# NVIDIA-NeMo/NeMo

Hardware: AMD Instinct MI355X
Metric: audio-sec/s training throughput, Conformer-CTC-Large @ 1/2/4/8 MI355X (higher is better)
Workload: dtype bf16; 1 GPU; Conformer-CTC-Large bf16, batch=32x20s synthetic 16 kHz clips per GPU, 1xMI355X (BASELINE.json configs[1]); global_batch=32, parallelism=dp1

## Files before the change

### nemo_amd/csrc/attention.hip

```cpp
#include <stdlib.h>
#include "common.h"
#include "mi355x_asr.h"

typedef __attribute__((address_space(3))) void lds_void_t;
typedef const __attribute__((address_space(1))) void glb_void_t;
typedef __attribute__((ext_vector_type(4))) short s16x4;
typedef __attribute__((address_space(3))) s16x4 lds_s16x4_t;

typedef __attribute__((address_space(3))) const char lds_cchar_t;
__device__ __forceinline__ uint32_t lds_addr(const void* p) { return (uint32_t)(uintptr_t)(lds_cchar_t*)p; }

__device__ __forceinline__ void dma16(const void* src, const void* lds_base) {
  asm volatile("s_mov_b32 m0, %1\n\ts_nop 0\n\tglobal_load_lds_dwordx4 %0, off"
               :
               : "v"(src), "s"(__builtin_amdgcn_readfirstlane(lds_addr(lds_base)))
               : "memory");
}

__device__ __forceinline__ void dma4(const void* src, const void* lds_base) {
  asm volatile("s_mov_b32 m0, %1\n\ts_nop 0\n\tglobal_load_lds_dword %0, off"
               :
               : "v"(src), "s"(__builtin_amdgcn_readfirstlane(lds_addr(lds_base)))
               : "memory");
}

#define ABQ 128
#define ABK 32
#define ABAND (ABQ + ABK)
#define SG_LD 66
#define APRING 6

__device__ __forceinline__ uint32_t attn_key(const DropCfg& d, int b, int h) {
  return mix32(mix32(d.key ^ (uint32_t)(b * 0x632BE5AB)) + (uint32_t)h * 0x9E3779B9u);
}
#define ADROP_G 0x9E3779B9u
#define ADROP_KA 0x2C1B3Du
#define ADROP_KB 0x5A2D39u
__device__ __forceinline__ uint32_t adrop_rcode(uint32_t akey, uint32_t bi) { return mix32(akey + bi * 0x9E3779B9u); }
__device__ __forceinline__ uint32_t adrop_ccode(uint32_t bj) { return mix32(bj * 0x85EBCA6Bu + 0x165667B1u); }
__device__ __forceinline__ uint32_t adrop_seed(uint32_t x) { return __umul24(x, 0x846CA7u) + (x >> 13); }
__device__ __forceinline__ uint32_t adrop_y(uint32_t t) { return t ^ (t >> 15); }
__device__ __forceinline__ bool attn_keep(const DropCfg& d, uint32_t akey, int i, int j) {
  if (d.threshold == 0u) return true;
  const uint32_t seed = adrop_seed(adrop_rcode(akey, (uint32_t)i >> 2) ^ adrop_ccode((uint32_t)j >> 2));
  const uint32_t y = adrop_y(seed + (uint32_t)((i & 3) * 2 + ((j & 3) >> 1)) * ADROP_G);
  return __umul24(y, (j & 1) ? ADROP_KB : ADROP_KA) >= d.threshold;
}
__device__ __forceinline__ float attn_drop(const DropCfg& d, uint32_t akey, int i, int j) {
  return attn_keep(d, akey, i, j) ? d.scale : 0.f;
}

template <int ADK>
__device__ __forceinline__ int a_off(int r, int chunk) { return r * ADK + ((chunk ^ ((r >> 1) & 7)) << 3); }

template <int ADK>
__device__ __forceinline__ void stage_rows(const bf16_t* base, long long ld, int row0, int rmax, bf16_t* lds, int nchunks) {
  constexpr int NCH = ADK / 8;
  const int wave = threadIdx.x >> 6;
  for (int q0 = 0; q0 < nchunks; q0 += 256) {
    const int q = q0 + threadIdx.x;
    if (q0 + wave * 64 < nchunks) {
      const int r = q / NCH, ck = q % NCH;
      const int gck = ck ^ ((r >> 1) & 7);
      int gr = row0 + r;
      gr = gr < 0 ? 0 : (gr > rmax ? rmax : gr);
      const bf16_t* src = base + __mul24(gr, (int)ld) + gck * 8;
      bf16_t* dst = lds + (q0 + wave * 64) * 8;
      dma16(src, dst);
    }
  }
}
template <int ADK>
__device__ __forceinline__ void stage_v(const bf16_t* base, long long ld, int row0, int rmax, bf16_t* lds) {
  constexpr int NCH = ADK / 8;
  const int wave = threadIdx.x >> 6;
#pragma unroll
  for (int q0 = 0; q0 < 32 * NCH; q0 += 256) {
    const int q = q0 + threadIdx.x;
    const int k = q / NCH, cp = q % NCH;
    const int c = cp ^ ((k & 3) << 1);
    int gr = row0 + k;
    gr = gr > rmax ? rmax : gr;
    const bf16_t* src = base + __mul24(gr, (int)ld) + c * 8;
    bf16_t* dst = lds + (q0 + wave * 64) * 8;
    dma16(src, dst);
  }
}
template <int ADK>
__device__ __forceinline__ bf16x8 vt_frag(const bf16_t* vt, int dv0, int s, int lane) {
  const int t = lane & 15, g4 = (lane >> 4) & 1, lh = lane >> 5;
  const int col = dv0 + g4 * 16 + (t & 3) * 4;
  union { bf16x8 v; s16x4 h[2]; } u;
#pragma unroll
  for (int r = 0; r < 2; ++r) {
    const int krow = 16 * s + 8 * r + 4 * lh + (t >> 2);
    const int off = krow * ADK + (((col >> 3) ^ ((krow & 3) << 1)) << 3) + (col & 7);
    u.h[r] = __builtin_amdgcn_ds_read_tr16_b64_v4i16((lds_s16x4_t*)(vt + off));
  }
  return u.v;
}

__device__ __forceinline__ bf16x8 pack8(const float* v) {
  union { bf16x8 v; uint32_t w[4]; } u;
#pragma unroll
  for (int j = 0; j < 4; ++j) u.w[j] = pack_bf2(v[2 * j], v[2 * j + 1]);
  return u.v;
}

template <int NKK>
__device__ __forceinline__ void load_q(const bf16_t* qrow, const float* bias, bf16x8 (&out)[NKK], bool valid, int lh) {
#pragma unroll
  for (int kk = 0; kk < NKK; ++kk) {
    float v[8];
    const int k0 = kk * 16 + lh * 8;
    if (valid) {
      const u32x4 t = *reinterpret_cast<const u32x4*>(qrow + k0);
#pragma unroll
      for (int j = 0; j < 4; ++j) { v[2 * j] = __uint_as_float(t[j] << 16); v[2 * j + 1] = __uint_as_float(t[j] & 0xffff0000u); }
#pragma unroll
      for (int j = 0; j < 8; ++j) v[j] += bias[k0 + j];
    } else {
#pragma unroll
      for (int j = 0; j < 8; ++j) v[j] = 0.f;
    }
    out[kk] = pack8(v);
  }
}

template <int ADK>
__global__ __launch_bounds__(256, ADK == 64 ? 2 : 1) void relpos_flash_fwd_kernel(const bf16_t* __restrict__ qkv, long long ldq,
                                                                  const bf16_t* __restrict__ pos, long long ldp,
                                                                  const float* __restrict__ bias_u, const float* __restrict__ bias_v,
                                                                  const long long* __restrict__ len, bf16_t* __restrict__ ctx,
                                                                  bf16_t* __restrict__ ctx_lo, long long ldo,
                                                                  float* __restrict__ lse, int B, int H, int T,
                                                                  int Tp, float scale, DropCfg drop,
                                                                  const long long* __restrict__ cu) {
  drop_resolve(drop);
  constexpr int NKK = ADK / 16, NDT = ADK / 32, NCH = ADK / 8;
  __shared__ __attribute__((aligned(16))) bf16_t s_k2[2][ABK * ADK];
  __shared__ __attribute__((aligned(16))) bf16_t s_v2[2][ABK * ADK];
  __shared__ __attribute__((aligned(16))) bf16_t s_p[APRING * 32 * ADK];
  __shared__ __attribute__((aligned(16))) float s_g[4][32 * SG_LD];

  const int b = blockIdx.z, h = blockIdx.y;
  const int i0_blk = blockIdx.x * ABQ;
  const int lane = threadIdx.x & 63, wave = __builtin_amdgcn_readfirstlane(threadIdx.x >> 6);
  const int q = lane & 31, lh = lane >> 5;
  const int i = i0_blk + wave * 32 + q;
  const int L = (int)min((long long)T, len[b]);
  const bool qvalid = i < L;
  const int P = 2 * T - 1;
  const long long row0 = cu ? cu[b] : (long long)b * T;
  const int Tr = cu ? L : T;
  const int Trc = Tr > 0 ? Tr - 1 : 0;

  if (cu && i0_blk >= L) {
    if (lse && lh == 0 && i < T) lse[((long long)b * H + h) * T + i] = 0.f;
    return;
  }
  const bf16_t* qbase = qkv + row0 * ldq + h * ADK;
  const bf16_t* kbase = qbase + (ldq / 3);
  const bf16_t* vbase = qbase + 2 * (ldq / 3);
  const bf16_t* pbase = pos + h * ADK;

  bf16x8 qu[NKK], qv[NKK];
  load_q<NKK>(qbase + (long long)(i < Tr ? i : Trc) * ldq, bias_u + h * ADK, qu, i < Tr, lh);
  load_q<NKK>(qbase + (long long)(i < Tr ? i : Trc) * ldq, bias_v + h * ADK, qv, i < Tr, lh);

  f32x16 o[NDT];
#pragma unroll
  for (int t = 0; t < NDT; ++t)
#pragma unroll
    for (int r = 0; r < 16; ++r) o[t][r] = 0.f;
  float m_run = -INFINITY, l_run = 0.f;
  float* sg = s_g[wave];
  const uint32_t akey = attn_key(drop, b, h);
  const uint32_t arow = adrop_rcode(akey, (uint32_t)i >> 2), erow = (uint32_t)(i & 3) * (2u * ADROP_G);
  const float c2 = scale * 1.4426950408889634f, tau = 8.f / c2;

  const int nkt = (L + ABK - 1) / ABK;
  const int c0 = T - 1 - (i0_blk + ABQ - 1);
  if (nkt > 0) {
    stage_rows<ADK>(kbase, ldq, 0, Trc, s_k2[0], ABK * NCH);
    stage_v<ADK>(vbase, ldq, 0, Trc, s_v2[0]);
    stage_rows<ADK>(pbase, ldp, c0, P - 1, s_p, ABAND * NCH);
  }
  for (int kt = 0; kt < nkt; ++kt) {
    const int j0 = kt * ABK;
    asm volatile("s_waitcnt vmcnt(0)" ::: "memory");
    __syncthreads();
    if (kt + 1 < nkt) {
      stage_rows<ADK>(kbase, ldq, j0 + ABK, Trc, s_k2[(kt + 1) & 1], ABK * NCH);
      stage_v<ADK>(vbase, ldq, j0 + ABK, Trc, s_v2[(kt + 1) & 1]);
      stage_rows<ADK>(pbase, ldp, c0 + 32 * (kt + 5), P - 1, s_p + ((kt + 5) % APRING) * (32 * ADK), 32 * NCH);
    }
    const bf16_t* s_k = s_k2[kt & 1];
    const bf16_t* s_v = s_v2[kt & 1];
    const int slot0 = (kt + 3 - wave) % APRING, slot1 = (kt + 4 - wave) % APRING;

    f32x16 acc_s, acc_g[2];
#pragma unroll
    for (int r = 0; r < 16; ++r) { acc_s[r] = 0.f; acc_g[0][r] = 0.f; acc_g[1][r] = 0.f; }
#pragma unroll
    for (int kk = 0; kk < NKK; ++kk) {
      const bf16x8 kf = *reinterpret_cast<const bf16x8*>(s_k + a_off<ADK>(q, kk * 2 + lh));
      acc_s = __builtin_amdgcn_mfma_f32_32x32x16_bf16(kf, qu[kk], acc_s, 0, 0, 0);
#pragma unroll
      for (int gt = 0; gt < 2; ++gt) {
        const bf16x8 pf = *reinterpret_cast<const bf16x8*>(s_p + a_off<ADK>((gt ? slot1 : slot0) * 32 + q, kk * 2 + lh));
        acc_g[gt] = __builtin_amdgcn_mfma_f32_32x32x16_bf16(pf, qv[kk], acc_g[gt], 0, 0, 0);
      }
    }
#pragma unroll
    for (int gt = 0; gt < 2; ++gt)
#pragma unroll
      for (int r = 0; r < 16; ++r) sg[q * SG_LD + 32 * gt + (r & 3) + 8 * (r >> 2) + 4 * lh] = acc_g[gt][r];
    asm volatile("s_waitcnt lgkmcnt(0)" ::: "memory");
    float s[16];
    float mx = -INFINITY;
    if (j0 + ABK <= L) {
#pragma unroll
      for (int r = 0; r < 16; ++r) {
        const int rho = (r & 3) + 8 * (r >> 2) + 4 * lh;
        s[r] = acc_s[r] + sg[q * SG_LD + rho + 31 - q];
        mx = fmaxf(mx, s[r]);
      }
    } else {
#pragma unroll
      for (int r = 0; r < 16; ++r) {
        const int rho = (r & 3) + 8 * (r >> 2) + 4 * lh;
        const float bd = sg[q * SG_LD + rho + 31 - q];
        const bool ok = qvalid && (j0 + rho) < L;
        s[r] = ok ? acc_s[r] + bd : -INFINITY;
        mx = fmaxf(mx, s[r]);
      }
    }
    asm volatile("s_waitcnt lgkmcnt(0)" ::: "memory");
    mx = fmaxf(mx, __shfl_xor(mx, 32, 64));
    if (__builtin_amdgcn_ballot_w64(mx > m_run + tau) != 0ull) {
      const float m_new = fmaxf(m_run, mx);
      const float alpha = (m_new == -INFINITY) ? 1.f : __builtin_amdgcn_exp2f((m_run - m_new) * c2);
      l_run *= alpha;
#pragma unroll
      for (int r = 0; r < 16; ++r) { o[0][r] *= alpha; o[1][r] *= alpha; }
      m_run = m_new;
    }
    const float mc = (m_run == -INFINITY) ? 0.f : m_run * c2;
    float rs = 0.f;
#pragma unroll
    for (int r = 0; r < 16; ++r) { s[r] = __builtin_amdgcn_exp2f(fmaf(s[r], c2, -mc)); rs += s[r]; }
    rs += __shfl_xor(rs, 32, 64);
    l_run += rs;
    if (drop.threshold != 0u) {
      const uint32_t bj0 = (uint32_t)(j0 >> 2);
#pragma unroll
      for (int g = 0; g < 4; ++g) {
        const uint32_t cc0 = adrop_ccode(bj0 + 2 * g), cc1 = adrop_ccode(bj0 + 2 * g + 1);
        const uint32_t seed = adrop_seed(arow ^ (lh ? cc1 : cc0)) + erow;
#pragma unroll
        for (int cp = 0; cp < 2; ++cp) {
          const uint32_t y = adrop_y(seed + cp * ADROP_G);
          s[4 * g + 2 * cp] = __umul24(y, ADROP_KA) >= drop.threshold ? s[4 * g + 2 * cp] : 0.f;
          s[4 * g + 2 * cp + 1] = __umul24(y, ADROP_KB) >= drop.threshold ? s[4 * g + 2 * cp + 1] : 0.f;
        }
      }
    }
#pragma unroll
    for (int st = 0; st < 2; ++st) {
      const bf16x8 pb = pack8(&s[8 * st]);
#pragma unroll
      for (int dvt = 0; dvt < NDT; ++dvt) {
        const bf16x8 vf = vt_frag<ADK>(s_v, dvt * 32, st, lane);
        o[dvt] = __builtin_amdgcn_mfma_f32_32x32x16_bf16(vf, pb, o[dvt], 0, 0, 0);
      }
    }
  }

  const float inv = (qvalid && l_run > 0.f) ? (drop.threshold != 0u ? drop.scale : 1.f) / l_run : 0.f;
  __syncthreads();
  if (lse && lh == 0 && i < T) lse[((long long)b * H + h) * T + i] = qvalid ? m_run * scale + __logf(l_run) : 0.f;
#pragma unroll
  for (int half = 0; half < NDT / 2; ++half) {
#pragma unroll
  for (int dvt = 0; dvt < 2; ++dvt)
#pragma unroll
    for (int r = 0; r < 16; ++r) sg[q * SG_LD + dvt * 32 + (r & 3) + 8 * (r >> 2) + 4 * lh] = o[2 * half + dvt][r] * inv;
  asm volatile("s_waitcnt lgkmcnt(0)" ::: "memory");
#pragma unroll
  for (int it = 0; it < 4; ++it) {
    const int row = it * 8 + (lane >> 3), c8 = (lane & 7) * 8, co = half * 64 + c8;
    const int ii = i0_blk + wave * 32 + row;
    if (ii < Tr) {
      float v[8];
#pragma unroll
      for (int j = 0; j < 8; ++j) v[j] = sg[row * SG_LD + c8 + j];
      u32x4 t = {pack_bf2(v[0], v[1]), pack_bf2(v[2], v[3]), pack_bf2(v[4], v[5]), pack_bf2(v[6], v[7])};
      *reinterpret_cast<u32x4*>(ctx + (row0 + ii) * ldo + h * ADK + co) = t;
      if (ctx_lo) {
        float lo[8];
#pragma unroll
        for (int j = 0; j < 4; ++j) {
          lo[2 * j] = v[2 * j] - __uint_as_float(t[j] << 16);
          lo[2 * j + 1] = v[2 * j + 1] - __uint_as_float(t[j] & 0xffff0000u);
        }
        u32x4 tl = {pack_bf2(lo[0], lo[1]), pack_bf2(lo[2], lo[3]), pack_bf2(lo[4], lo[5]), pack_bf2(lo[6], lo[7])};
        *reinterpret_cast<u32x4*>(ctx_lo + (row0 + ii) * ldo + h * ADK + co) = tl;
      }
    }
  }
  asm volatile("s_waitcnt lgkmcnt(0)" ::: "memory");
  }
}

template <bool QB, int ADK>
__global__ __launch_bounds__(256) void attn_delta_kernel(const bf16_t* __restrict__ dO, const bf16_t* __restrict__ O,
                                                         const bf16_t* __restrict__ O_lo, float* __restrict__ delta,
                                                         const bf16_t* __restrict__ qkv, long long ldq,
                                                         const float* __restrict__ bias_u, const float* __restrict__ bias_v,
                                                         bf16_t* __restrict__ qu, bf16_t* __restrict__ qv, int B,
                                                         int H, int T, int d, const long long* __restrict__ len,
                                                         const long long* __restrict__ cu) {
  const int lane = threadIdx.x & 63;
  const long long prow = blockIdx.x * 4LL + (threadIdx.x >> 6);
  if (prow >= (long long)B * T) return;
  const int b = (int)(prow / T), i = (int)(prow - (long long)b * T);
  const bool rvalid = !cu || i < (int)min((long long)T, len[b]);
  const long long row = cu ? cu[b] + (rvalid ? i : 0) : prow;
  for (int c0 = 0; c0 < d; c0 += 512) {
    const int c = c0 + lane * 8;
    float acc = 0.f;
    if (QB && c < d && rvalid) {
      float q8[8], u8[8], v8[8], o1[8], o2[8];
      VecIO<bf16_t>::load(qkv + row * ldq + c, q8);
      VecIO<float>::load(bias_u + c, u8); VecIO<float>::load(bias_u + c + 4, &u8[4]);
      VecIO<float>::load(bias_v + c, v8); VecIO<float>::load(bias_v + c + 4, &v8[4]);
#pragma unroll
      for (int j = 0; j < 8; ++j) { o1[j] = q8[j] + u8[j]; o2[j] = q8[j] + v8[j]; }
      VecIO<bf16_t>::store(qu + row * d + c, o1);
      VecIO<bf16_t>::store(qv + row * d + c, o2);
    }
    if (c < d && rvalid) {
      const u32x4 a = *reinterpret_cast<const u32x4*>(dO + row * d + c);
      const u32x4 o = *reinterpret_cast<const u32x4*>(O + row * d + c);
#pragma unroll
      for (int j = 0; j < 4; ++j) {
        acc += __uint_as_float(a[j] << 16) * __uint_as_float(o[j] << 16);
        acc += __uint_as_float(a[j] & 0xffff0000u) * __uint_as_float(o[j] & 0xffff0000u);
      }
      if (O_lo) {
        const u32x4 l = *reinterpret_cast<const u32x4*>(O_lo + row * d + c);
        float acl = 0.f;
#pragma unroll
        for (int j = 0; j < 4; ++j) {
          acl += __uint_as_float(a[j] << 16) * __uint_as_float(l[j] << 16);
          acl += __uint_as_float(a[j] & 0xffff0000u) * __uint_as_float(l[j] & 0xffff0000u);
        }
        acc += acl;
      }
    }
    acc += __shfl_xor(acc, 1, 64); acc += __shfl_xor(acc, 2, 64); acc += __shfl_xor(acc, 4, 64);
    if (ADK == 128) acc += __shfl_xor(acc, 8, 64);
    const int h = c / ADK;
    if ((lane & (ADK / 8 - 1)) == 0 && c < d) delta[((long long)b * H + h) * T + i] = acc;
  }
}

template <int ADK>
__device__ __forceinline__ bf16x8 tr_frag(const bf16_t* img, int ra, int rb, int col0, int lane) {
  const int t = lane & 15, g4 = (lane >> 4) & 1;
  const int col = col0 + g4 * 16 + (t & 3) * 4;
  union { bf16x8 v; s16x4 h[2]; } u;
  const int r0 = ra + (t >> 2), r1 = rb + (t >> 2);
  u.h[0] = __builtin_amdgcn_ds_read_tr16_b64_v4i16((lds_s16x4_t*)(img + r0 * ADK + ((((col >> 3) ^ ((r0 >> 1) & 7))) << 3) + (col & 7)));
  u.h[1] = __builtin_amdgcn_ds_read_tr16_b64_v4i16((lds_s16x4_t*)(img + r1 * ADK + ((((col >> 3) ^ ((r1 >> 1) & 7))) << 3) + (col & 7)));
  return u.v;
}
template <int NKK>
__device__ __forceinline__ void load_rows(const bf16_t* rowp, bf16x8 (&out)[NKK], bool valid, int lh) {
#pragma unroll
  for (int kk = 0; kk < NKK; ++kk) {
    union { bf16x8 v; u32x4 w; } u;
    u.w = (u32x4){0u, 0u, 0u, 0u};
    if (valid) u.w = *reinterpret_cast<const u32x4*>(rowp + kk * 16 + lh * 8);
    out[kk] = u.v;
  }
}

template <int ADK>
__global__ __launch_bounds__(256, ADK == 64 ? 2 : 1) void relpos_flash_bwd_dq_kernel(
    const bf16_t* __restrict__ qu_g, const bf16_t* __restrict__ qv_g, const bf16_t* __restrict__ qkv, long long ldq,
    const bf16_t* __restrict__ pos, long long ldp, const long long* __restrict__ len, const bf16_t* __restrict__ dO,
    const float* __restrict__ lse, const float* __restrict__ delta, bf16_t* __restrict__ dqu_out,
    bf16_t* __restrict__ dqv_out, bf16_t* __restrict__ ds_out, bf16_t* __restrict__ dq_out, long long ld_dq,
    float* __restrict__ cs_partial, int B, int H, int T, int d, float scale, DropCfg drop,
    const long long* __restrict__ cu) {
  drop_resolve(drop);
  constexpr int NKK = ADK / 16, NDT = ADK / 32, NCH = ADK / 8;
  __shared__ __attribute__((aligned(16))) bf16_t s_k2[2][ABK * ADK];
  __shared__ __attribute__((aligned(16))) bf16_t s_v[ABK * ADK];
  __shared__ __attribute__((aligned(16))) bf16_t s_p[APRING * 32 * ADK];
  __shared__ __attribute__((aligned(16))) float s_g[4][32 * SG_LD];
  __shared__ __attribute__((aligned(16))) bf16_t s_carry[4][32 * 32];

  const int b = blockIdx.z, h = blockIdx.y;
  const int i0_blk = blockIdx.x * ABQ;
  const int lane = threadIdx.x & 63, wave = __builtin_amdgcn_readfirstlane(threadIdx.x >> 6);
  const int q = lane & 31, lh = lane >> 5;
  const int i = i0_blk + wave * 32 + q;
  const int L = (int)min((long long)T, len[b]);
  const bool qvalid = i < L;
  const int P = 2 * T - 1;
  const long long row0 = cu ? cu[b] : (long long)b * T;
  const int Tr = cu ? L : T;
  const int Trc = Tr > 0 ? Tr - 1 : 0;
  if (cu && i0_blk >= L) {
    if (dq_out && cs_partial && threadIdx.x < 2 * ADK) {
      const int uv = threadIdx.x / ADK, c = threadIdx.x % ADK;
      cs_partial[((long long)b * gridDim.x + blockIdx.x) * (2 * d) + uv * d + h * ADK + c] = 0.f;
    }
    return;
  }
  const long long rowi = row0 + (i < Tr ? i : Trc);

  const bf16_t* kbase = qkv + row0 * ldq + h * ADK + (ldq / 3);
  const bf16_t* vbase = kbase + (ldq / 3);
  const bf16_t* pbase = pos + h * ADK;

  bf16x8 qu[NKK], qv[NKK], dof[NKK];
  load_rows<NKK>(qu_g + rowi * d + h * ADK, qu, i < Tr, lh);
  load_rows<NKK>(qv_g + rowi * d + h * ADK, qv, i < Tr, lh);
  load_rows<NKK>(dO + rowi * d + h * ADK, dof, i < Tr, lh);
  float lse_i = qvalid ? lse[((long long)b * H + h) * T + i] : 1e30f;
  float dlt_i = qvalid ? delta[((long long)b * H + h) * T + i] : 0.f;
#pragma unroll
  for (int kk = 0; kk < NKK; ++kk) { asm volatile("" : "+v"(qu[kk])); asm volatile("" : "+v"(qv[kk])); asm volatile("" : "+v"(dof[kk])); }
  asm volatile("" : "+v"(lse_i), "+v"(dlt_i));

  f32x16 dqu[NDT], dqv[NDT];
#pragma unroll
  for (int t = 0; t < NDT; ++t)
#pragma unroll
    for (int r = 0; r < 16; ++r) { dqu[t][r] = 0.f; dqv[t][r] = 0.f; }
  float* sg = s_g[wave];
  const uint32_t akey = attn_key(drop, b, h);
  const uint32_t arow = adrop_rcode(akey, (uint32_t)i >> 2), erow = (uint32_t)(i & 3) * (2u * ADROP_G);
  const float c2 = scale * 1.4426950408889634f, lse2 = lse_i * 1.4426950408889634f;
  const float ks = drop.threshold != 0u ? drop.scale * scale : scale, dls = dlt_i * scale;

  const int nkt = (L + ABK - 1) / ABK;
  const int nT = (T + 31) / 32, itile = blockIdx.x * 4 + wave;
  const bool xw = ds_out != nullptr && itile < nT;
  bf16_t* xbase = ds_out + ((((long long)h * B + b) * nT + itile) * (nT + 1)) * 1024;
  u32x4* carry = reinterpret_cast<u32x4*>(s_carry[wave]);
  if (xw) { carry[lane] = (u32x4){0u, 0u, 0u, 0u}; carry[64 + lane] = (u32x4){0u, 0u, 0u, 0u}; }
  const int c0 = T - 1 - (i0_blk + ABQ - 1);
  if (nkt > 0) {
    stage_rows<ADK>(kbase, ldq, 0, Trc, s_k2[0], ABK * NCH);
    stage_rows<ADK>(vbase, ldq, 0, Trc, s_v, ABK * NCH);
    stage_rows<ADK>(pbase, ldp, c0, P - 1, s_p, ABAND * NCH);
  }
  for (int kt = 0; kt < nkt; ++kt) {
    const int j0 = kt * ABK;
    asm volatile("s_waitcnt vmcnt(0)" ::: "memory");
    __syncthreads();
    if (kt + 1 < nkt) {
      stage_rows<ADK>(kbase, ldq, j0 + ABK, Trc, s_k2[(kt + 1) & 1], ABK * NCH);
      stage_rows<ADK>(pbase, ldp, c0 + 32 * (kt + 5), P - 1, s_p + ((kt + 5) % APRING) * (32 * ADK), 32 * NCH);
    }
    const bf16_t* s_k = s_k2[kt & 1];
    const int slot0 = (kt + 3 - wave) % APRING, slot1 = (kt + 4 - wave) % APRING;

    f32x16 acc_s, acc_g[2], acc_dp;
#pragma unroll
    for (int r = 0; r < 16; ++r) { acc_s[r] = 0.f; acc_g[0][r] = 0.f; acc_g[1][r] = 0.f; acc_dp[r] = 0.f; }
#pragma unroll
    for (int kk = 0; kk < NKK; ++kk) {
      const bf16x8 kf = *reinterpret_cast<const bf16x8*>(s_k + a_off<ADK>(q, kk * 2 + lh));
      acc_s = __builtin_amdgcn_mfma_f32_32x32x16_bf16(kf, qu[kk], acc_s, 0, 0, 0);
      const bf16x8 vf = *reinterpret_cast<const bf16x8*>(s_v + a_off<ADK>(q, kk * 2 + lh));
      acc_dp = __builtin_amdgcn_mfma_f32_32x32x16_bf16(vf, dof[kk], acc_dp, 0, 0, 0);
#pragma unroll
      for (int gt = 0; gt < 2; ++gt) {
        const bf16x8 pf = *reinterpret_cast<const bf16x8*>(s_p + a_off<ADK>((gt ? slot1 : slot0) * 32 + q, kk * 2 + lh));
        acc_g[gt] = __builtin_amdgcn_mfma_f32_32x32x16_bf16(pf, qv[kk], acc_g[gt], 0, 0, 0);
      }
    }
    if (kt + 1 < nkt) {
      __syncthreads();
      stage_rows<ADK>(vbase, ldq, j0 + ABK, Trc, s_v, ABK * NCH);
    }
#pragma unroll
    for (int gt = 0; gt < 2; ++gt)
#pragma unroll
      for (int r = 0; r < 16; ++r) sg[q * SG_LD + 32 * gt + (r & 3) + 8 * (r >> 2) + 4 * lh] = acc_g[gt][r];
    asm volatile("s_waitcnt lgkmcnt(0)" ::: "memory");
    float ds[16];
    if (j0 + ABK <= L) {
#pragma unroll
      for (int r = 0; r < 16; ++r) {
        const int rho = (r & 3) + 8 * (r >> 2) + 4 * lh;
        ds[r] = __builtin_amdgcn_exp2f(fmaf(acc_s[r] + sg[q * SG_LD + rho + 31 - q], c2, -lse2));
      }
    } else {
#pragma unroll
      for (int r = 0; r < 16; ++r) {
        const int rho = (r & 3) + 8 * (r >> 2) + 4 * lh;
        const float bd = sg[q * SG_LD + rho + 31 - q];
        ds[r] = (j0 + rho) < L ? __builtin_amdgcn_exp2f(fmaf(acc_s[r] + bd, c2, -lse2)) : 0.f;
      }
    }
    asm volatile("s_waitcnt lgkmcnt(0)" ::: "memory");
    if (drop.threshold != 0u) {
      const uint32_t bj0 = (uint32_t)(j0 >> 2);
#pragma unroll
      for (int g = 0; g < 4; ++g) {
        const uint32_t cc0 = adrop_ccode(bj0 + 2 * g), cc1 = adrop_ccode(bj0 + 2 * g + 1);
        const uint32_t seed = adrop_seed(arow ^ (lh ? cc1 : cc0)) + erow;
#pragma unroll
        for (int cp = 0; cp < 2; ++cp) {
          const uint32_t y = adrop_y(seed + cp * ADROP_G);
          const int r0 = 4 * g + 2 * cp;
          const float x0 = __umul24(y, ADROP_KA) >= drop.threshold ? acc_dp[r0] : 0.f;
          const float x1 = __umul24(y, ADROP_KB) >= drop.threshold ? acc_dp[r0 + 1] : 0.f;
          ds[r0] *= fmaf(x0, ks, -dls);
          ds[r0 + 1] *= fmaf(x1, ks, -dls);
        }
      }
    } else {
#pragma unroll
      for (int r = 0; r < 16; ++r) ds[r] *= fmaf(acc_dp[r], ks, -dls);
    }
#pragma unroll
    for (int st = 0; st < 2; ++st) {
      const bf16x8 db = pack8(&ds[8 * st]);
#pragma unroll
      for (int dkt = 0; dkt < NDT; ++dkt) {
        const bf16x8 kt_f = tr_frag<ADK>(s_k, 16 * st + 4 * lh, 16 * st + 8 + 4 * lh, dkt * 32, lane);
        dqu[dkt] = __builtin_amdgcn_mfma_f32_32x32x16_bf16(kt_f, db, dqu[dkt], 0, 0, 0);
      }
    }
    {
      const float2 z = make_float2(0.f, 0.f);
#pragma unroll
      for (int w2 = 0; w2 < 16; ++w2) *reinterpret_cast<float2*>(sg + q * SG_LD + 32 * lh + 2 * w2) = z;
    }
    asm volatile("s_waitcnt lgkmcnt(0)" ::: "memory");
#pragma unroll
    for (int r = 0; r < 16; ++r) sg[q * SG_LD + (r & 3) + 8 * (r >> 2) + 4 * lh + 31 - q] = ds[r];
    asm volatile("s_waitcnt lgkmcnt(0)" ::: "memory");
#pragma unroll
    for (int s4 = 0; s4 < 4; ++s4) {
      float gv[8];
#pragma unroll
      for (int e = 0; e < 8; ++e) gv[e] = sg[q * SG_LD + 16 * s4 + 8 * lh + e];
      const bf16x8 gb = pack8(gv);
#pragma unroll
      for (int dkt = 0; dkt < NDT; ++dkt) {
        const int ra = (s4 < 2 ? slot0 : slot1) * 32 + 16 * (s4 & 1) + 8 * lh;
        const bf16x8 pt_f = tr_frag<ADK>(s_p, ra, ra + 4, dkt * 32, lane);
        dqv[dkt] = __builtin_amdgcn_mfma_f32_32x32x16_bf16(pt_f, gb, dqv[dkt], 0, 0, 0);
      }
    }
    asm volatile("s_waitcnt lgkmcnt(0)" ::: "memory");
    if (xw) {
#pragma unroll
      for (int it2 = 0; it2 < 2; ++it2) {
        const int row = it2 * 16 + (lane >> 2), c8 = (lane & 3) * 8;
        float lo[8], hi[8];
#pragma unroll
        for (int e = 0; e < 8; ++e) { lo[e] = sg[row * SG_LD + c8 + e]; hi[e] = sg[row * SG_LD + 32 + c8 + e]; }
        const u32x4 cw = carry[it2 * 64 + lane];
        u32x4 t = {pack_bf2(lo[0], lo[1]) | cw.x, pack_bf2(lo[2], lo[3]) | cw.y, pack_bf2(lo[4], lo[5]) | cw.z,
                   pack_bf2(lo[6], lo[7]) | cw.w};
        *reinterpret_cast<u32x4*>(xbase + (long long)kt * 1024 + it2 * 512 + lane * 8) = t;
        carry[it2 * 64 + lane] = (u32x4){pack_bf2(hi[0], hi[1]), pack_bf2(hi[2], hi[3]), pack_bf2(hi[4], hi[5]), pack_bf2(hi[6], hi[7])};
      }
      asm volatile("s_waitcnt lgkmcnt(0)" ::: "memory");
    }
  }
  if (xw) {
#pragma unroll
    for (int it2 = 0; it2 < 2; ++it2)
      *reinterpret_cast<u32x4*>(xbase + (long long)nkt * 1024 + it2 * 512 + lane * 8) = carry[it2 * 64 + lane];
  }

  __syncthreads();
  constexpr int NH = NDT / 2;
  float keep[NH][4][8], cs[2][NH][8];
#pragma unroll
  for (int hf = 0; hf < NH; ++hf)
#pragma unroll
    for (int j = 0; j < 8; ++j) { cs[0][hf][j] = 0.f; cs[1][hf][j] = 0.f; }
#pragma unroll
  for (int pass = 0; pass < 2; ++pass) {
    bf16_t* outp = pass == 0 ? dqu_out : dqv_out;
#pragma unroll
    for (int hf = 0; hf < NH; ++hf) {
#pragma unroll
    for (int dkt = 0; dkt < 2; ++dkt)
#pragma unroll
      for (int r = 0; r < 16; ++r)
        sg[q * SG_LD + dkt * 32 + (r & 3) + 8 * (r >> 2) + 4 * lh] = qvalid ? (pass == 0 ? dqu[2 * hf + dkt][r] : dqv[2 * hf + dkt][r]) : 0.f;
    asm volatile("s_waitcnt lgkmcnt(0)" ::: "memory");
#pragma unroll
    for (int it = 0; it < 4; ++it) {
      const int row = it * 8 + (lane >> 3), c8 = (lane & 7) * 8, co = hf * 64 + c8;
      const int ii = i0_blk + wave * 32 + row;
      if (ii < Tr) {
        float v[8];
#pragma unroll
        for (int j = 0; j < 8; ++j) v[j] = sg[row * SG_LD + c8 + j];
        if (outp) {
          u32x4 t = {pack_bf2(v[0], v[1]), pack_bf2(v[2], v[3]), pack_bf2(v[4], v[5]), pack_bf2(v[6], v[7])};
          *reinterpret_cast<u32x4*>(outp + (row0 + ii) * d + h * ADK + co) = t;
        }
        if (dq_out) {
#pragma unroll
          for (int j = 0; j < 8; ++j) cs[pass][hf][j] += v[j];
          if (pass == 0) {
#pragma unroll
            for (int j = 0; j < 8; ++j) keep[hf][it][j] = v[j];
          } else {
#pragma unroll
            for (int j = 0; j < 8; ++j) v[j] += keep[hf][it][j];
            u32x4 t = {pack_bf2(v[0], v[1]), pack_bf2(v[2], v[3]), pack_bf2(v[4], v[5]), pack_bf2(v[6], v[7])};
            *reinterpret_cast<u32x4*>(dq_out + (row0 + ii) * ld_dq + h * ADK + co) = t;
          }
        }
      }
    }
    asm volatile("s_waitcnt lgkmcnt(0)" ::: "memory");
    }
  }
  if (dq_out && cs_partial) {
#pragma unroll
    for (int pass = 0; pass < 2; ++pass)
#pragma unroll
      for (int hf = 0; hf < NH; ++hf)
#pragma unroll
      for (int j = 0; j < 8; ++j) {
        float v = cs[pass][hf][j];
        v += __shfl_xor(v, 8, 64); v += __shfl_xor(v, 16, 64); v += __shfl_xor(v, 32, 64);
        cs[pass][hf][j] = v;
      }
    if (lane < 8) {
#pragma unroll
      for (int pass = 0; pass < 2; ++pass)
#pragma unroll
        for (int hf = 0; hf < NH; ++hf)
#pragma unroll
        for (int j = 0; j < 8; ++j) sg[pass * ADK + hf * 64 + lane * 8 + j] = cs[pass][hf][j];
    }
    __syncthreads();
    if (threadIdx.x < 2 * ADK) {
      const int uv = threadIdx.x / ADK, c = threadIdx.x % ADK;
      const float t = (s_g[0][threadIdx.x] + s_g[1][threadIdx.x]) + (s_g[2][threadIdx.x] + s_g[3][threadIdx.x]);
      cs_partial[((long long)b * gridDim.x + blockIdx.x) * (2 * d) + uv * d + h * ADK + c] = t;
    }
  }
}

template <int ADK>
__global__ __launch_bounds__(256, ADK == 64 ? 2 : 1) void relpos_flash_bwd_dkv_kernel(
    const bf16_t* __restrict__ qu_g, const bf16_t* __restrict__ qv_g, const bf16_t* __restrict__ qkv, long long ldq,
    const bf16_t* __restrict__ pos, long long ldp, const long long* __restrict__ len, const bf16_t* __restrict__ dO,
    const float* __restrict__ lse, const float* __restrict__ delta, bf16_t* __restrict__ dqkv, long long ldd, int B, int H,
    int T, int Tp, int d, float scale, DropCfg drop, const long long* __restrict__ cu) {
  drop_resolve(drop);
  constexpr int NKK = ADK / 16, NDT = ADK / 32, NCH = ADK / 8;
  constexpr int STAGE_BYTES = 2 * 3 * 32 * ADK * 2 + APRING * 32 * ADK * 2 + 2 * 2 * 32 * 4;
  constexpr int OUT_BYTES = 4 * 32 * SG_LD * 4;
  __shared__ __attribute__((aligned(16))) char s_raw[STAGE_BYTES > OUT_BYTES ? STAGE_BYTES : OUT_BYTES];
  bf16_t* const s_q3 = reinterpret_cast<bf16_t*>(s_raw);
  bf16_t* const s_p = reinterpret_cast<bf16_t*>(s_raw + 2 * 3 * 32 * ADK * 2);
  float* const s_ld = reinterpret_cast<float*>(s_raw + 2 * 3 * 32 * ADK * 2 + APRING * 32 * ADK * 2);

  const int b = blockIdx.z, h = blockIdx.y;
  const int j0_blk = blockIdx.x * ABQ;
  const int lane = threadIdx.x & 63, wave = __builtin_amdgcn_readfirstlane(threadIdx.x >> 6);
  const int q = lane & 31, lh = lane >> 5;
  const int j = j0_blk + wave * 32 + q;
  const int L = (int)min((long long)T, len[b]);
  const bool kvalid = j < L;
  const int P = 2 * T - 1;
  const long long row0 = cu ? cu[b] : (long long)b * T;
  const int Tr = cu ? L : T;
  const int Trc = Tr > 0 ? Tr - 1 : 0;
  if (cu && j0_blk >= L) return;
  const long long rowj = row0 + (j < Tr ? j : Trc);
  const bf16_t* kbase = qkv + (ldq / 3) + h * ADK;
  const bf16_t* pbase = pos + h * ADK;
  const uint32_t akey = attn_key(drop, b, h);
  const uint32_t acol = adrop_ccode((uint32_t)j >> 2), ecol = (uint32_t)((j & 3) >> 1) * ADROP_G;
  const uint32_t klane = (j & 1) ? ADROP_KB : ADROP_KA;
  const float dscale = drop.threshold != 0u ? drop.scale : 1.f;

  bf16x8 kf[NKK], vf[NKK];
  load_rows<NKK>(kbase + rowj * ldq, kf, j < Tr, lh);
  load_rows<NKK>(kbase + (ldq / 3) + rowj * ldq, vf, j < Tr, lh);

#pragma unroll
  for (int kk = 0; kk < NKK; ++kk) { asm volatile("" : "+v"(kf[kk])); asm volatile("" : "+v"(vf[kk])); }
  f32x16 dk_acc[NDT], dv_acc[NDT];
#pragma unroll
  for (int t = 0; t < NDT; ++t)
#pragma unroll
    for (int r = 0; r < 16; ++r) { dk_acc[t][r] = 0.f; dv_acc[t][r] = 0.f; }

  const int nqt = (L + 31) / 32;
  const bf16_t* qub = qu_g + row0 * d + h * ADK;
  const bf16_t* qvb = qv_g + row0 * d + h * ADK;
  const bf16_t* dob = dO + row0 * d + h * ADK;
  const int cb0 = T - 1 + j0_blk - 31;
  auto stage_q = [&](int i0, int buf) {
    bf16_t* dst = s_q3 + buf * (3 * 32 * ADK);
    stage_rows<ADK>(qub, d, i0, Trc, dst, 32 * NCH);
    stage_rows<ADK>(qvb, d, i0, Trc, dst + 32 * ADK, 32 * NCH);
    stage_rows<ADK>(dob, d, i0, Trc, dst + 2 * 32 * ADK, 32 * NCH);
    if (wave == 0) {
      int ii = i0 + (lane & 31);
      ii = ii < T ? ii : T - 1;
      dma4((lane < 32 ? lse : delta) + ((long long)b * H + h) * T + ii, s_ld + buf * 64);
    }
  };
  if (nqt > 0) {
    stage_q(0, 0);
    stage_rows<ADK>(pbase, ldp, cb0, P - 1, s_p, ABAND * NCH);
  }
  for (int qt = 0; qt < nqt; ++qt) {
    const int i0 = qt * 32;
    asm volatile("s_waitcnt vmcnt(0)" ::: "memory");
    __syncthreads();
    if (qt + 1 < nqt) {
      stage_q(i0 + 32, (qt + 1) & 1);
      stage_rows<ADK>(pbase, ldp, cb0 - 32 * (qt + 1), P - 1, s_p + ((6 * 1024 - (qt + 1)) % APRING) * (32 * ADK), 32 * NCH);
    }
    const bf16_t* s_qu = s_q3 + (qt & 1) * (3 * 32 * ADK);
    const bf16_t* s_qv = s_qu + 32 * ADK;
    const bf16_t* s_do = s_qu + 2 * 32 * ADK;
    const float* s_lse = s_ld + (qt & 1) * 64;
    const float* s_dlt = s_lse + 32;
    const int slot0 = (6 * 1024 - qt + wave) % APRING, slot1 = (6 * 1024 - qt + wave + 1) % APRING;

    f32x16 acc_s, acc_g[2], acc_dp;
#pragma unroll
    for (int r = 0; r < 16; ++r) { acc_s[r] = 0.f; acc_g[0][r] = 0.f; acc_g[1][r] = 0.f; acc_dp[r] = 0.f; }
#pragma unroll
    for (int kk = 0; kk < NKK; ++kk) {
      const bf16x8 quf = *reinterpret_cast<const bf16x8*>(s_qu + a_off<ADK>(q, kk * 2 + lh));
      acc_s = __builtin_amdgcn_mfma_f32_32x32x16_bf16(quf, kf[kk], acc_s, 0, 0, 0);
      const bf16x8 dof = *reinterpret_cast<const bf16x8*>(s_do + a_off<ADK>(q, kk * 2 + lh));
      acc_dp = __builtin_amdgcn_mfma_f32_32x32x16_bf16(dof, vf[kk], acc_dp, 0, 0, 0);
      const bf16x8 qvf = *reinterpret_cast<const bf16x8*>(s_qv + a_off<ADK>(q, kk * 2 + lh));
#pragma unroll
      for (int ct = 0; ct < 2; ++ct) {
        const bf16x8 pf = *reinterpret_cast<const bf16x8*>(s_p + a_off<ADK>((ct ? slot1 : slot0) * 32 + q, kk * 2 + lh));
        acc_g[ct] = __builtin_amdgcn_mfma_f32_32x32x16_bf16(qvf, pf, acc_g[ct], 0, 0, 0);
      }
    }
    float pd[16], ds[16];
    uint32_t w4[4] = {0xffffffffu, 0xffffffffu, 0xffffffffu, 0xffffffffu};
#pragma unroll
    for (int r = 0; r < 16; ++r) {
      if ((r & 3) == 0 && drop.threshold != 0u) {
        const uint32_t rr0 = adrop_rcode(akey, (uint32_t)(i0 >> 2) + 2 * (r >> 2));
        const uint32_t rr1 = adrop_rcode(akey, (uint32_t)(i0 >> 2) + 2 * (r >> 2) + 1);
        const uint32_t seed = adrop_seed((lh ? rr1 : rr0) ^ acol) + ecol;
#pragma unroll
        for (int c = 0; c < 4; ++c) w4[c] = __umul24(adrop_y(seed + c * (2u * ADROP_G)), klane);
      }
      const int rho = (r & 3) + 8 * (r >> 2) + 4 * lh;
      const int sl = 31 + q - rho;
      const float g0 = __shfl(acc_g[0][r], lh * 32 + (sl & 31), 64);
      const float g1 = __shfl(acc_g[1][r], lh * 32 + (sl & 31), 64);
      const float bd = sl < 32 ? g0 : g1;
      const int ii = i0 + rho;
      const bool ok = kvalid && ii < L;
      const float p = ok ? __expf((acc_s[r] + bd) * scale - s_lse[rho]) : 0.f;
      const bool keep = w4[r & 3] >= drop.threshold;
      pd[r] = keep ? p : 0.f;
      ds[r] = p * fmaf(keep ? acc_dp[r] : 0.f, dscale, -s_dlt[rho]);
    }
#pragma unroll
    for (int st = 0; st < 2; ++st) {
      const bf16x8 pb = pack8(&pd[8 * st]);
      const bf16x8 db = pack8(&ds[8 * st]);
      const int ra = 16 * st + 4 * lh, rb = 16 * st + 8 + 4 * lh;
#pragma unroll
      for (int t2 = 0; t2 < NDT; ++t2) {
        const bf16x8 dot_f = tr_frag<ADK>(s_do, ra, rb, t2 * 32, lane);
        dv_acc[t2] = __builtin_amdgcn_mfma_f32_32x32x16_bf16(dot_f, pb, dv_acc[t2], 0, 0, 0);
        const bf16x8 qut_f = tr_frag<ADK>(s_qu, ra, rb, t2 * 32, lane);
        dk_acc[t2] = __builtin_amdgcn_mfma_f32_32x32x16_bf16(qut_f, db, dk_acc[t2], 0, 0, 0);
      }
    }
  }
  __syncthreads();

  float* st_ = reinterpret_cast<float*>(s_raw) + wave * (32 * SG_LD);
#pragma unroll
  for (int pass = 0; pass < 2 * (NDT / 2); ++pass) {
    const int kind = pass / (NDT / 2), hf = pass % (NDT / 2);
#pragma unroll
    for (int t2 = 0; t2 < 2; ++t2)
#pragma unroll
      for (int r = 0; r < 16; ++r)
        st_[q * SG_LD + t2 * 32 + (r & 3) + 8 * (r >> 2) + 4 * lh] =
            kind == 0 ? dk_acc[2 * hf + t2][r] * scale : dv_acc[2 * hf + t2][r] * dscale;
    asm volatile("s_waitcnt lgkmcnt(0)" ::: "memory");
#pragma unroll
    for (int it = 0; it < 4; ++it) {
      const int row = it * 8 + (lane >> 3), c8 = (lane & 7) * 8;
      const int jj = j0_blk + wave * 32 + row;
      if (jj < Tr) {
        float v[8];
#pragma unroll
        for (int e = 0; e < 8; ++e) v[e] = st_[row * SG_LD + c8 + e];
        u32x4 t = {pack_bf2(v[0], v[1]), pack_bf2(v[2], v[3]), pack_bf2(v[4], v[5]), pack_bf2(v[6], v[7])};
        *reinterpret_cast<u32x4*>(dqkv + (row0 + jj) * ldd + (kind + 1) * (ldd / 3) + h * ADK + hf * 64 + c8) = t;
      }
    }
    asm volatile("s_waitcnt lgkmcnt(0)" ::: "memory");
  }
}

__device__ __forceinline__ bf16x8 tr_frag32(const bf16_t* img, int ra, int rb, int lane) {
  const int t = lane & 15, g4 = (lane >> 4) & 1;
  const int col = g4 * 16 + (t & 3) * 4;
  union { bf16x8 v; s16x4 h[2]; } u;
  u.h[0] = __builtin_amdgcn_ds_read_tr16_b64_v4i16((lds_s16x4_t*)(img + (ra + (t >> 2)) * 32 + col));
  u.h[1] = __builtin_amdgcn_ds_read_tr16_b64_v4i16((lds_s16x4_t*)(img + (rb + (t >> 2)) * 32 + col));
  return u.v;
}

template <int ADK>
__global__ __launch_bounds__(256, ADK == 64 ? 2 : 1) void relpos_flash_bwd_dpos_kernel(
    const bf16_t* __restrict__ qv_g, const bf16_t* __restrict__ x_g, const long long* __restrict__ len,
    float* __restrict__ dpos, long long ldd, float* __restrict__ partial, int B, int H, int T, int d, int bchunk,
    const long long* __restrict__ cu) {
  constexpr int NDT = ADK / 32, NCH = ADK / 8;
  __shared__ __attribute__((aligned(16))) bf16_t s_x[4][2][2 * 1024];
  __shared__ __attribute__((aligned(16))) bf16_t s_qv[4][2][32 * ADK];

  const int nT = (T + 31) / 32;
  const int dg = 2 * (int)blockIdx.x - (nT - 1);
  const int h = blockIdx.y;
  const int b_begin = blockIdx.z * bchunk, b_end = min(B, b_begin + bchunk);
  const int lane = threadIdx.x & 63, wave = __builtin_amdgcn_readfirstlane(threadIdx.x >> 6);
  const int q = lane & 31, lh = lane >> 5;
  const int P = 2 * T - 1;
  const int cmin = T - 32 + 32 * dg;
  const int it_lo = max(0, -dg - 1), it_hi = min(nT, nT - dg + 1);

  f32x16 dp_acc[2][NDT];
#pragma unroll
  for (int t = 0; t < NDT; ++t)
#pragma unroll
    for (int r = 0; r < 16; ++r) { dp_acc[0][t][r] = 0.f; dp_acc[1][t][r] = 0.f; }

  const int npairs = it_hi - it_lo;
  const int nitems = (b_end - b_begin) * npairs;
  auto issue = [&](int b, int it, int buf) {
    const int s0 = it + dg;
    const int sl0 = min(max(s0, 0), nT), sl1 = min(max(s0 + 1, 0), nT);
    const bf16_t* base = x_g + ((((long long)h * B + b) * nT + it) * (nT + 1)) * 1024;
    bf16_t* sx = s_x[wave][buf];
    bf16_t* sqv = s_qv[wave][buf];
#pragma unroll
    for (int k2 = 0; k2 < 2; ++k2) {
      dma16((base + sl0 * 1024 + k2 * 512 + lane * 8), (sx + k2 * 512));
      dma16((base + sl1 * 1024 + k2 * 512 + lane * 8), (sx + 1024 + k2 * 512));
    }
    const int Lb = cu ? (int)min((long long)T, len[b]) : T;
    const bf16_t* qb = qv_g + (cu ? (Lb > 0 ? cu[b] : 0LL) : (long long)b * T) * d + h * ADK;
    const int grmax = Lb > 0 ? Lb - 1 : 0;
#pragma unroll
    for (int k4 = 0; k4 < 32 * NCH / 64; ++k4) {
      const int cq = k4 * 64 + lane;
      const int r = cq / NCH, ck = cq % NCH;
      int gr = 32 * it + r;
      gr = gr > grmax ? grmax : gr;
      dma16((qb + __mul24(gr, d) + ((ck ^ ((r >> 1) & 7)) << 3)), (sqv + k4 * 512));
    }
  };
  auto advance = [&](int& b, int& it, int steps) {
    it += steps;
// ... 275 lines not shown
```

Measured before the change: 17820 audio-sec/s.

## Reuse overlapping positional band tile across key iterations in rel-pos attention

In both forward and backward relative-position attention kernels, the positional-band product for slot1 in one key tile equals the slot0 product of the next tile. The change computes it once per iteration and carries it forward, in a parity-swapped scratch buffer in the forward pass and a g_carry register in the backward pass, which cuts the band MFMAs roughly in half. The backward pass also merges the dS export with the dQv accumulation by carrying packed half-tiles in LDS and adding a trailing MFMA pass after the loop. This adds more complex indexing (wraparound reads in the forward pass), extra registers and a tail step, so correctness depends on the carry logic being right at tile boundaries.

```diff
diff --git a/nemo_amd/csrc/attention.hip b/nemo_amd/csrc/attention.hip
--- a/nemo_amd/csrc/attention.hip
+++ b/nemo_amd/csrc/attention.hip
@@ -198,41 +198,60 @@
     const bf16_t* s_k = s_k2[kt & 1];
     const bf16_t* s_v = s_v2[kt & 1];
     const int slot0 = (kt + 3 - wave) % APRING, slot1 = (kt + 4 - wave) % APRING;
-
-    f32x16 acc_s, acc_g[2];
-#pragma unroll
-    for (int r = 0; r < 16; ++r) { acc_s[r] = 0.f; acc_g[0][r] = 0.f; acc_g[1][r] = 0.f; }
+    const int par = (kt + 3 - wave) & 1;
+
+    f32x16 acc_s, acc_g;
+    if (kt == 0) {
+#pragma unroll
+      for (int r = 0; r < 16; ++r) acc_g[r] = 0.f;
+#pragma unroll
+      for (int kk = 0; kk < NKK; ++kk) {
+        const bf16x8 pf = *reinterpret_cast<const bf16x8*>(s_p + a_off<ADK>(slot0 * 32 + q, kk * 2 + lh));
+        acc_g = __builtin_amdgcn_mfma_f32_32x32x16_bf16(pf, qv[kk], acc_g, 0, 0, 0);
+      }
+#pragma unroll
+      for (int r = 0; r < 16; ++r) sg[q * SG_LD + 32 * par + (r & 3) + 8 * (r >> 2) + 4 * lh] = acc_g[r];
+    }
+#pragma unroll
+    for (int r = 0; r < 16; ++r) { acc_s[r] = 0.f; acc_g[r] = 0.f; }
 #pragma unroll
     for (int kk = 0; kk < NKK; ++kk) {
       const bf16x8 kf = *reinterpret_cast<const bf16x8*>(s_k + a_off<ADK>(q, kk * 2 + lh));
       acc_s = __builtin_amdgcn_mfma_f32_32x32x16_bf16(kf, qu[kk], acc_s, 0, 0, 0);
-#pragma unroll
-      for (int gt = 0; gt < 2; ++gt) {
-        const bf16x8 pf = *reinterpret_cast<const bf16x8*>(s_p + a_off<ADK>((gt ? slot1 : slot0) * 32 + q, kk * 2 + lh));
-        acc_g[gt] = __builtin_amdgcn_mfma_f32_32x32x16_bf16(pf, qv[kk], acc_g[gt], 0, 0, 0);
-      }
-    }
-#pragma unroll
-    for (int gt = 0; gt < 2; ++gt)
-#pragma unroll
-      for (int r = 0; r < 16; ++r) sg[q * SG_LD + 32 * gt + (r & 3) + 8 * (r >> 2) + 4 * lh] = acc_g[gt][r];
+      const bf16x8 pf = *reinterpret_cast<const bf16x8*>(s_p + a_off<ADK>(slot1 * 32 + q, kk * 2 + lh));
+      acc_g = __builtin_amdgcn_mfma_f32_32x32x16_bf16(pf, qv[kk], acc_g, 0, 0, 0);
+    }
+#pragma unroll
+    for (int r = 0; r < 16; ++r) sg[q * SG_LD + 32 * (par ^ 1) + (r & 3) + 8 * (r >> 2) + 4 * lh] = acc_g[r];
     asm volatile("s_waitcnt lgkmcnt(0)" ::: "memory");
+    float bd[16];
+    {
+      const float* rd = sg + q * SG_LD + 31 - q + 32 * par;
+      if (par == 0) {
+#pragma unroll
+        for (int r = 0; r < 16; ++r) bd[r] = rd[(r & 3) + 8 * (r >> 2) + 4 * lh];
+      } else {
+#pragma unroll
+        for (int r = 0; r < 16; ++r) {
+          const int rho = (r & 3) + 8 * (r >> 2) + 4 * lh;
+          bd[r] = rd[rho > q ? rho - 64 : rho];
+        }
+      }
+    }
     float s[16];
     float mx = -INFINITY;
     if (j0 + ABK <= L) {
 #pragma unroll
       for (int r = 0; r < 16; ++r) {
-        const int rho = (r & 3) + 8 * (r >> 2) + 4 * lh;
-        s[r] = acc_s[r] + sg[q * SG_LD + rho + 31 - q];
+        s[r] = acc_s[r] + bd[r];
         mx = fmaxf(mx, s[r]);
       }
     } else {
 #pragma unroll
       for (int r = 0; r < 16; ++r) {
         const int rho = (r & 3) + 8 * (r >> 2) + 4 * lh;
-        const float bd = sg[q * SG_LD + rho + 31 - q];
         const bool ok = qvalid && (j0 + rho) < L;
-        s[r] = ok ? acc_s[r] + bd : -INFINITY;
+        s[r] = ok ? acc_s[r] + bd[r] : -INFINITY;
         mx = fmaxf(mx, s[r]);
       }
     }
@@ -452,8 +471,9 @@
   const int nT = (T + 31) / 32, itile = blockIdx.x * 4 + wave;
   const bool xw = ds_out != nullptr && itile < nT;
   bf16_t* xbase = ds_out + ((((long long)h * B + b) * nT + itile) * (nT + 1)) * 1024;
-  u32x4* carry = reinterpret_cast<u32x4*>(s_carry[wave]);
-  if (xw) { carry[lane] = (u32x4){0u, 0u, 0u, 0u}; carry[64 + lane] = (u32x4){0u, 0u, 0u, 0u}; }
+  u32x4* carry = reinterpret_cast<u32x4*>(s_carry[wave]) + lane;
+  carry[0] = (u32x4){0u, 0u, 0u, 0u}; carry[64] = (u32x4){0u, 0u, 0u, 0u};
+  f32x16 g_carry;
   const int c0 = T - 1 - (i0_blk + ABQ - 1);
   if (nkt > 0) {
     stage_rows<ADK>(kbase, ldq, 0, Trc, s_k2[0], ABK * NCH);
@@ -471,29 +491,37 @@
     const bf16_t* s_k = s_k2[kt & 1];
     const int slot0 = (kt + 3 - wave) % APRING, slot1 = (kt + 4 - wave) % APRING;
 
-    f32x16 acc_s, acc_g[2], acc_dp;
-#pragma unroll
-    for (int r = 0; r < 16; ++r) { acc_s[r] = 0.f; acc_g[0][r] = 0.f; acc_g[1][r] = 0.f; acc_dp[r] = 0.f; }
+    f32x16 acc_s, acc_g, acc_dp;
+    if (kt == 0) {
+#pragma unroll
+      for (int r = 0; r < 16; ++r) g_carry[r] = 0.f;
+#pragma unroll
+      for (int kk = 0; kk < NKK; ++kk) {
+        const bf16x8 pf = *reinterpret_cast<const bf16x8*>(s_p + a_off<ADK>(slot0 * 32 + q, kk * 2 + lh));
+        g_carry = __builtin_amdgcn_mfma_f32_32x32x16_bf16(pf, qv[kk], g_carry, 0, 0, 0);
+      }
+    }
+#pragma unroll
+    for (int r = 0; r < 16; ++r) { acc_s[r] = 0.f; acc_g[r] = 0.f; acc_dp[r] = 0.f; }
 #pragma unroll
     for (int kk = 0; kk < NKK; ++kk) {
       const bf16x8 kf = *reinterpret_cast<const bf16x8*>(s_k + a_off<ADK>(q, kk * 2 + lh));
       acc_s = __builtin_amdgcn_mfma_f32_32x32x16_bf16(kf, qu[kk], acc_s, 0, 0, 0);
       const bf16x8 vf = *reinterpret_cast<const bf16x8*>(s_v + a_off<ADK>(q, kk * 2 + lh));
       acc_dp = __builtin_amdgcn_mfma_f32_32x32x16_bf16(vf, dof[kk], acc_dp, 0, 0, 0);
-#pragma unroll
-      for (int gt = 0; gt < 2; ++gt) {
-        const bf16x8 pf = *reinterpret_cast<const bf16x8*>(s_p + a_off<ADK>((gt ? slot1 : slot0) * 32 + q, kk * 2 + lh));
-        acc_g[gt] = __builtin_amdgcn_mfma_f32_32x32x16_bf16(pf, qv[kk], acc_g[gt], 0, 0, 0);
-      }
+      const bf16x8 pf = *reinterpret_cast<const bf16x8*>(s_p + a_off<ADK>(slot1 * 32 + q, kk * 2 + lh));
+      acc_g = __builtin_amdgcn_mfma_f32_32x32x16_bf16(pf, qv[kk], acc_g, 0, 0, 0);
     }
     if (kt + 1 < nkt) {
       __syncthreads();
       stage_rows<ADK>(vbase, ldq, j0 + ABK, Trc, s_v, ABK * NCH);
     }
 #pragma unroll
-    for (int gt = 0; gt < 2; ++gt)
-#pragma unroll
-      for (int r = 0; r < 16; ++r) sg[q * SG_LD + 32 * gt + (r & 3) + 8 * (r >> 2) + 4 * lh] = acc_g[gt][r];
+    for (int r = 0; r < 16; ++r) {
+      sg[q * SG_LD + (r & 3) + 8 * (r >> 2) + 4 * lh] = g_carry[r];
+      sg[q * SG_LD + 32 + (r & 3) + 8 * (r >> 2) + 4 * lh] = acc_g[r];
+    }
+    g_carry = acc_g;
     asm volatile("s_waitcnt lgkmcnt(0)" ::: "memory");
     float ds[16];
     if (j0 + ABK <= L) {
@@ -550,39 +578,45 @@
     for (int r = 0; r < 16; ++r) sg[q * SG_LD + (r & 3) + 8 * (r >> 2) + 4 * lh + 31 - q] = ds[r];
     asm volatile("s_waitcnt lgkmcnt(0)" ::: "memory");
 #pragma unroll
-    for (int s4 = 0; s4 < 4; ++s4) {
+    for (int s2 = 0; s2 < 2; ++s2) {
       float gv[8];
 #pragma unroll
-      for (int e = 0; e < 8; ++e) gv[e] = sg[q * SG_LD + 16 * s4 + 8 * lh + e];
-      const bf16x8 gb = pack8(gv);
+      for (int e = 0; e < 8; ++e) gv[e] = sg[q * SG_LD + 16 * s2 + 8 * lh + e];
+      union { bf16x8 v; u32x4 w; } gb;
+      gb.v = pack8(gv);
+      const u32x4 cw = carry[64 * s2];
+      gb.w.x |= cw.x; gb.w.y |= cw.y; gb.w.z |= cw.z; gb.w.w |= cw.w;
+      if (xw) *reinterpret_cast<u32x4*>(xbase + (long long)kt * 1024 + q * 32 + (2 * s2 + lh) * 8) = gb.w;
 #pragma unroll
       for (int dkt = 0; dkt < NDT; ++dkt) {
-        const int ra = (s4 < 2 ? slot0 : slot1) * 32 + 16 * (s4 & 1) + 8 * lh;
+        const int ra = slot0 * 32 + 16 * s2 + 8 * lh;
         const bf16x8 pt_f = tr_frag<ADK>(s_p, ra, ra + 4, dkt * 32, lane);
-        dqv[dkt] = __builtin_amdgcn_mfma_f32_32x32x16_bf16(pt_f, gb, dqv[dkt], 0, 0, 0);
-      }
+        dqv[dkt] = __builtin_amdgcn_mfma_f32_32x32x16_bf16(pt_f, gb.v, dqv[dkt], 0, 0, 0);
+      }
+#pragma unroll
+      for (int e = 0; e < 8; ++e) gv[e] = sg[q * SG_LD + 32 + 16 * s2 + 8 * lh + e];
+      gb.v = pack8(gv);
+      carry[64 * s2] = gb.w;
     }
     asm volatile("s_waitcnt lgkmcnt(0)" ::: "memory");
-    if (xw) {
-#pragma unroll
-      for (int it2 = 0; it2 < 2; ++it2) {
-        const int row = it2 * 16 + (lane >> 2), c8 = (lane & 3) * 8;
-        float lo[8], hi[8];
-#pragma unroll
-        for (int e = 0; e < 8; ++e) { lo[e] = sg[row * SG_LD + c8 + e]; hi[e] = sg[row * SG_LD + 32 + c8 + e]; }
-        const u32x4 cw = carry[it2 * 64 + lane];
-        u32x4 t = {pack_bf2(lo[0], lo[1]) | cw.x, pack_bf2(lo[2], lo[3]) | cw.y, pack_bf2(lo[4], lo[5]) | cw.z,
-                   pack_bf2(lo[6], lo[7]) | cw.w};
-        *reinterpret_cast<u32x4*>(xbase + (long long)kt * 1024 + it2 * 512 + lane * 8) = t;
-        carry[it2 * 64 + lane] = (u32x4){pack_bf2(hi[0], hi[1]), pack_bf2(hi[2], hi[3]), pack_bf2(hi[4], hi[5]), pack_bf2(hi[6], hi[7])};
-      }
-      asm volatile("s_waitcnt lgkmcnt(0)" ::: "memory");
+  }
+  if (nkt > 0) {
+    const int slotl = (nkt + 3 - wave) % APRING;
+#pragma unroll
+    for (int s2 = 0; s2 < 2; ++s2) {
+      union { bf16x8 v; u32x4 w; } gb;
+      gb.w = carry[64 * s2];
+#pragma unroll
+      for (int dkt = 0; dkt < NDT; ++dkt) {
+        const int ra = slotl * 32 + 16 * s2 + 8 * lh;
+        const bf16x8 pt_f = tr_frag<ADK>(s_p, ra, ra + 4, dkt * 32, lane);
+        dqv[dkt] = __builtin_amdgcn_mfma_f32_32x32x16_bf16(pt_f, gb.v, dqv[dkt], 0, 0, 0);
+      }
     }
   }
   if (xw) {
 #pragma unroll
-    for (int it2 = 0; it2 < 2; ++it2)
-      *reinterpret_cast<u32x4*>(xbase + (long long)nkt * 1024 + it2 * 512 + lane * 8) = carry[it2 * 64 + lane];
+    for (int s2 = 0; s2 < 2; ++s2) *reinterpret_cast<u32x4*>(xbase + (long long)nkt * 1024 + q * 32 + (2 * s2 + lh) * 8) = carry[64 * s2];
   }
 
   __syncthreads();
```

Result: no change. 17970 audio-sec/s, median of 6 (+0.8%).
